# Costava/heightmap-ray-marcher

Measured on AMD Instinct MI355X. Metric: ray-steps/s at 3840x2160, 4096^2 heightmap, higher is better.
Workload: dtype f64; 1 GPU; C3: 4096x4096 heightmap, 3840x2160, spherical hfov 180, step_dist 0.25, grid_width 1; ray_steps_per_frame=1197030646, rays_per_frame=8294400, hits_per_frame=1006074, parallelism=1 GPU, launches back to back on one stream

## Files before the change

### heightmap-ray-marcher_amd/__init__.py

```python
from .lib import (
    Camera, Config, HmrmError, Scene, SceneParams, Stats,
    Ray, RayHit, TraceParams, SegmentParams, Sun, Water, CellMapParams, CellRect, GeometryPlanes, LightPlanes, MAP_TOWARDS_POINT, MAP_WEIGHT, MAP_DIFFUSE, MAP_NO_SHADOWS, RAY_END, TRACE_INTERIOR, SHADE_DIFFUSE, SHADE_NO_SHADOWS, RAY_DTYPE, RAY_HIT_DTYPE, RAY_MISS, RAY_HIT, RAY_CAPPED, MAX_RAYS, as_rays,
    PERSPECTIVE, SPHERICAL, ORTHOGRAPHIC, NEAREST, BILINEAR, NEAREST_F32,
    HMRM_OK, HMRM_E_ARG, HMRM_E_IO, HMRM_E_IMAGE, HMRM_E_CONFIG, HMRM_E_DEVICE, HMRM_E_NOTERM,
    EXPORTED_SYMBOLS, LIB_PATH, NO_PROBE, AA_FACTORS, aa_flags,
    band_local_rows, debug_frame, degrees_to_rads, device_count, image_load, image_load_memory, kernel_src_sha,
    last_error, mip_layout, level_state, calibrate, pick_kernel, plan_order, rcp_error, orbit_camera, orbit_frame_owner, png_encode, record_orbit, record_orbit_multi, record_orbit_shaded, record_orbit_baked, record_orbit_water, LIGHT_U8, LIGHT_U16, WATER_OWN_COLOR, WATER_BAKED, Haze, HAZE_SKY, HAZE_LINEAR, HAZE_EXP, HAZE_EXP2, MAX_HAZE_ENTRIES, haze_table, MAX_VIEWS, camera_array, views_tables, shade_flags, map_flags, sky_directions, render_multi, set_device, write_png, write_ppm, write_pfm,
)
from . import synth
```

### heightmap-ray-marcher_amd/csrc/api_aux.cpp

```cpp
#include <algorithm>
#include <cstdlib>
#include <cstring>
#include <fstream>
#include <new>
#include <sstream>

#include "api_internal.hpp"
#include "config.hpp"
#include "host_pool.hpp"
#include "image_io.hpp"

struct hmrm_config {
	hmrm::Config cfg;
	std::string log_cache, warn_cache;
};

extern "C" {

int hmrm_debug_kernel_choice(const hmrm_scene *s) {
	if (!s) return fail(HMRM_E_ARG, "NULL argument");
	std::lock_guard<std::mutex> lk(const_cast<hmrm_scene *>(s)->mu);
	if (s->knobs.kernel != 0) return s->knobs.kernel;
	return s->choice.use_group ? (s->choice.with_records ? 3 : 1) : 0;
}
// ... 335 lines not shown
	if (cam->projection == HMRM_SPHERICAL) {
		double *cc = tables, *cs = tables + W, *rs = tables + 2 * W, *rc2 = tables + 2 * W + H;
		const int nc = cam->width, nr = cam->height;
		hmrm::parallel_ranges(nc + nr, 1024, [&](int b, int e) {
			if (b < nc) hmrm::fill_col_tables(hc, b, std::min(e, nc), cc, cs);
			if (e > nc) hmrm::fill_row_tables(hc, std::max(b, nc) - nc, e - nc, rs, rc2);
		});
	}
	double *o = out25;
	for (int i = 0; i < 3; ++i) *o++ = f.cam[i];
	for (int i = 0; i < 3; ++i) *o++ = f.upper_left[i];
	for (int i = 0; i < 3; ++i) *o++ = f.plane_right[i];
	for (int i = 0; i < 3; ++i) *o++ = f.plane_down[i];
	for (int i = 0; i < 3; ++i) *o++ = f.look[i];
	for (int i = 0; i < 3; ++i) *o++ = f.c0[i];
	for (int i = 0; i < 3; ++i) *o++ = f.c1[i];
	*o++ = f.nudge;
	*o++ = f.step_dist;
	*o++ = (double)f.grid_pow2;
	*o++ = f.inv_grid_width;
	return HMRM_OK;
}

int hmrm_debug_pick_kernel(int32_t forced, int32_t use_other, int32_t records_ok, int32_t scene_verdict, int32_t scene_with_records,
                           int32_t *with_records_after) {
	hmrm::KernelChoice choice;
	choice.use_group = scene_verdict != 0;
	choice.probed = choice.use_group;
	choice.with_records = scene_with_records != 0;
	const int k = hmrm::pick_fast_kernel(forced, use_other != 0, records_ok != 0, choice);
	if (with_records_after) *with_records_after = choice.with_records ? 1 : 0;
	return k;
}

int hmrm_debug_level_state(int32_t level, int32_t young, int32_t min_level, int32_t out[8]) {
	if (!out || level < 0 || level > hmrm::kMipLevels || min_level < 0 || min_level >= hmrm::kMipLevels)
		return fail(HMRM_E_ARG, "hmrm_debug_level_state: bad argument");
	const uint32_t b = (uint32_t)(hmrm::level_state_table() >> (8 * level)) & 0xffu;
	const int hs = (int)(b & 31u), back = (int)(b >> 5);
	const int lstep = hmrm::level_step(young ? 0 : -1);
	out[0] = hs;
	out[1] = back;
	out[2] = (back + 1) << hs;
	out[3] = lstep;
	out[4] = hmrm::level_coarser(level, lstep);
	out[5] = hmrm::level_finer(level, lstep, min_level);
// ... 31 lines not shown
```

### heightmap-ray-marcher_amd/csrc/api_internal.hpp

```cpp
#pragma once
#include <hip/hip_runtime_api.h>

#include <cstddef>
#include <cstdint>
#include <mutex>
#include <string>
#include <vector>

#include "../../include/hmrm.h"
#include "frame.hpp"
#include "launch_order.hpp"
#include "render.hpp"

#pragma GCC visibility push(hidden)
namespace hmrm {
extern thread_local std::string g_error;
int fail(int code, const std::string &msg);
}
using namespace hmrm;

#define HIP_TRY(expr)                                                                         \
	do {                                                                                      \
		hipError_t e_ = (expr);                                                               \
		if (e_ != hipSuccess)                                                                 \
			return fail(HMRM_E_DEVICE, std::string(#expr) + ": " + hipGetErrorString(e_));    \
	} while (0)

struct Knobs {
	int64_t step_cap = (int64_t)1 << 26;
	int kernel = 0;
	bool tile_order = true;
	int order_mode = 2;
	int diag_mode = 0;
	int min_level = -1;
	int finest_pause = -1;
	bool order_verbose = false;
	bool try_group = true;
	int min_plane_shift = 0;
	int seg_n = 0;
	int seg_b[3] = {0, 0, 0}, seg_c[3] = {0, 0, 0};
};

template <bool kPinned> struct Scratch {
	void *ptr = nullptr;
	size_t cap = 0;
	int reserve(size_t bytes) {
		if (bytes <= cap) return HMRM_OK;
		release();
		if (kPinned) HIP_TRY(hipHostMalloc(&ptr, bytes, hipHostMallocDefault));
		else HIP_TRY(hipMalloc(&ptr, bytes));
		cap = bytes;
		return HMRM_OK;
	}
	template <class T> T *as() const { return static_cast<T *>(ptr); }
	void release() {
		if (ptr) (void)(kPinned ? hipHostFree(ptr) : hipFree(ptr));
		ptr = nullptr;
		cap = 0;
	}
};
using DeviceScratch = Scratch<false>;
using PinnedScratch = Scratch<true>;

constexpr int kFrameSlots = 64;
constexpr int kMaxMeasRows = 512;
constexpr int kProbeAfterFrames = 6;
constexpr int kMaxStreamCtx = 32;

struct FrameSlot {
	bool valid = false;
	uint64_t stamp = 0;
	hmrm_camera cam{};
	hmrm_scene_params params{};
	uint64_t thr_max_bits = 0;
	hmrm::DevFrame frame{};
	std::vector<float> row_cost;
	double *d_tables = nullptr;
	double *h_tables = nullptr;
	hipEvent_t uploaded = nullptr;
	hmrm::OrderCalibration cal;
	int meas_rows = 0;
	hipEvent_t measured = nullptr;
};

struct ViewStage {
	double *h = nullptr, *h_dev = nullptr;
	size_t cap = 0;
	hipEvent_t uploaded = nullptr;
	bool used = false;
	uint64_t stamp = 0;
};
constexpr int kViewStages = 4;
constexpr size_t kMaxViewStagingBytes = (size_t)256 << 20;
struct RetiredArena {
	void *ptr;
	hipEvent_t after;
};

struct StreamCtx {
// ... 177 lines not shown
```

### heightmap-ray-marcher_amd/csrc/api_launch.cpp

```cpp
#include <algorithm>
#include <cstdio>
#include <cstring>

#include "api_internal.hpp"
#include "host_pool.hpp"

static_assert(sizeof(hmrm_sun) == 48, "hmrm_sun has padding");
static_assert(sizeof(hmrm_camera) == 3 * sizeof(int32_t) + 4 + 8 * sizeof(double), "hmrm_camera has padding");
static_assert(sizeof(hmrm_scene_params) == 6 * sizeof(double), "hmrm_scene_params has padding");
static_assert(HMRM_SHADE_DIFFUSE == hmrm::kShadeDiffuse && HMRM_SHADE_NO_SHADOWS == hmrm::kShadeNoShadows, "route_frame's flag bits");

namespace {

int ensure_meas(StreamCtx *c) {
	if (!c->d_meas) HIP_TRY(hipMalloc((void **)&c->d_meas, (size_t)kMaxMeasRows * hmrm::kMeasureStride * sizeof(unsigned long long)));
	if (!c->h_meas) {
		const size_t n = (size_t)kFrameSlots * 2 * kMaxMeasRows * sizeof(unsigned long long);
		HIP_TRY(hipHostMalloc((void **)&c->h_meas, n, hipHostMallocMapped));
		HIP_TRY(hipHostGetDevicePointer((void **)&c->h_meas_dev, c->h_meas, 0));
	}
	return HMRM_OK;
}

bool others_idle(hmrm_scene *s, StreamCtx *c) {
// ... 65 lines not shown
	s->choice.with_records = records_ok;
	if (records_ok) {
		const int rc_r = ensure_records(s);
		if (rc_r) return rc_r;
	}
	hmrm::FrameLaunch l = frame_launch(s, c, f, measured, req);
	for (int pass = 0; pass < 2; ++pass) {
		HIP_TRY(hmrm::launch_measure_init(measured.measure, tiles_y, c->stream));
		l.d_counters = c->d_counters + (pass ? 8 : 0);
		HIP_TRY(hmrm::launch_frame_march(l, pass == 0 ? hmrm::kLeaps : (records_ok ? hmrm::kRecords : hmrm::kPlainGroups)));
		HIP_TRY(hmrm::launch_measure_readback(measured.measure, s->h_probe_dev + (size_t)pass * 2 * kMaxMeasRows, tiles_y, c->stream));
	}
	HIP_TRY(hipEventRecord(s->probe_done, c->stream));
	s->probe_pending = true;
	s->choice.probed = true;
	s->probe_rows = tiles_y;
	s->probe_epoch_launched = s->probe_epoch;
	s->probe_ctx = c;
	c->probe_in_flight = true;
	return raise_measure_fence(s, c);
}

int launch_kernel(hmrm_scene *s, StreamCtx *c, const hmrm::DevFrame &f, const hmrm::RowMap &rows_in_order, const FrameRequest &req,
                  bool use_group) {
	const bool huge_side = s->map_w >= (1 << 24) || s->map_h >= (1 << 24);
	const LitFrame *lit = req.lit;
	const hmrm::FrameRoute route = hmrm::route_frame(s->knobs.kernel, huge_side, f.sampling, f.aa_shift != 0, req.interior == Interior::kByKernels,
	                                                 lit != nullptr, lit ? lit->shade_flags : 0u, lit && lit->sum);
	if (route.refused) return fail(HMRM_E_ARG, "maps with a side of 2^24 cells or more support nearest sampling only");
	hmrm::FrameLaunch l = frame_launch(s, c, f, rows_in_order, req);
	l.family = route.family;
	if (lit) {
		l.sun = lit->sun;
		if (route.ambient_sun) l.sun.ambient = 255u;
		l.primary_interior = lit->primary_interior;
		if (lit->sum) l.lsum = *lit->sum;
	}
	if (req.geom) {
		l.family = hmrm::kFrameGeometry;
		l.geo = *req.geom;
		l.primary_interior = req.interior != Interior::kNot;
	}
	if (req.baked) {
		l.family = hmrm::kFrameBaked;
		l.baked = *req.baked;
		l.primary_interior = req.interior != Interior::kNot;
	}
	if (req.water) {
		const bool aa = f.aa_shift != 0;
		if (req.baked) l.family = aa ? hmrm::kFrameWaterBakedAA : hmrm::kFrameWaterBaked;
		else l.family = aa ? hmrm::kFrameWaterAA : hmrm::kFrameWater;
		l.water = *req.water;
		l.primary_interior = req.interior != Interior::kNot;
		if (req.water_sun) {
// ... 8 lines not shown
	}
	if (route.literal) {
		HIP_TRY(hmrm::launch_frame_literal(l));
		return HMRM_OK;
	}
	const hmrm::FastKernel k = (hmrm::FastKernel)hmrm::pick_fast_kernel(s->knobs.kernel, use_group, f.sampling == 0 && s->d_records, s->choice);
	if (k == hmrm::kRecords) {
		const int rc_r = ensure_records(s);
		if (rc_r) return rc_r;
	}
	HIP_TRY(hmrm::launch_frame_march(l, k));
	return HMRM_OK;
}

int launch_maybe_measured(hmrm_scene *s, StreamCtx *c, const hmrm::DevFrame &f, FrameSlot *slot, hmrm::RowMap &rows_in_order, int tiles_y,
                          bool measure_now, const FrameRequest &req, bool use_group) {
	if (measure_now) {
		const int rc_m = ensure_meas(c);
		if (rc_m) return rc_m;
		if (!slot->measured) HIP_TRY(hipEventCreateWithFlags(&slot->measured, hipEventDisableTiming));
		rows_in_order.measure = c->d_meas;
		HIP_TRY(hmrm::launch_measure_init(rows_in_order.measure, tiles_y, c->stream));
	}
	const int rc_k = launch_kernel(s, c, f, rows_in_order, req, use_group);
	if (rc_k || !measure_now) return rc_k;
	const size_t idx = (size_t)(slot - c->slots);
	HIP_TRY(hmrm::launch_measure_readback(rows_in_order.measure, c->h_meas_dev + idx * 2 * kMaxMeasRows, tiles_y, c->stream));
	HIP_TRY(hipEventRecord(slot->measured, c->stream));
	slot->meas_rows = tiles_y;
	c->meas_owner = slot;
	return raise_measure_fence(s, c);
}

}

namespace hmrm {

int check_camera(const hmrm_camera *cam) {
	if (!cam) return fail(HMRM_E_ARG, "camera is NULL");
	if (cam->width <= 0 || cam->height <= 0) return fail(HMRM_E_ARG, "resolution must be positive");
	if ((int64_t)cam->width * cam->height > ((int64_t)1 << 31) / 4)
		return fail(HMRM_E_ARG, "resolution too large (the reference indexes the framebuffer with int)");
	if (cam->projection < 1 || cam->projection > 3) return fail(HMRM_E_ARG, "projection must be 1, 2 or 3");
	if (cam->sampling > HMRM_NEAREST_F32) return fail(HMRM_E_ARG, "sampling must be 0 (nearest), 1 (bilinear) or 2 (nearest, float heights)");
	return HMRM_OK;
}

// ... 67 lines not shown
		}
		hmrm::DevFrame &fr = slot->frame;
		hmrm::build_frame(hc, s->map_w, s->map_h, s->params.min_height, s->params.max_height, s->params.grid_width,
		                  &fr, nullptr, nullptr, nullptr, nullptr);
		if (cam->projection == HMRM_SPHERICAL) {
			const FrameSlot *row_donor = nullptr, *col_donor = nullptr;
			for (const FrameSlot &o : c->slots) {
				if (!o.valid || &o == slot || o.cam.projection != HMRM_SPHERICAL || !o.h_tables) continue;
				if (o.cam.width != cam->width || o.cam.hfov != cam->hfov) continue;
				if (!col_donor && o.cam.hang == cam->hang) col_donor = &o;
				if (!row_donor && o.cam.height == cam->height && o.cam.vang == cam->vang) row_donor = &o;
			}
			if (col_donor) memcpy(cc, col_donor->h_tables, 2 * W * sizeof(double));
			if (row_donor) memcpy(rs, row_donor->h_tables + 2 * (size_t)row_donor->cam.width, 2 * H * sizeof(double));
			const int nc = col_donor ? 0 : cam->width, nr = row_donor ? 0 : cam->height;
			if (nc + nr > 0)
				hmrm::parallel_ranges(nc + nr, 1024, [&](int b, int e) {
					if (b < nc) hmrm::fill_col_tables(hc, b, std::min(e, nc), cc, cs);
					if (e > nc) hmrm::fill_row_tables(hc, std::max(b, nc) - nc, e - nc, rs, rc);
				});
		}
		slot->row_cost.assign(((size_t)cam->height + kCostRows - 1) / kCostRows, 0.0f);
		hmrm::estimate_row_costs(fr, cc, cs, rs, rc, kCostRows, slot->row_cost.data());
		if (cam->projection == HMRM_SPHERICAL) {
			HIP_TRY(hmrm::launch_upload_tables(c->h_arena_dev + (slot->h_tables - c->h_arena), slot->d_tables, 2 * W + 2 * H, c->stream));
			HIP_TRY(hipEventRecord(slot->uploaded, c->stream));
			fr.col_cos_ha = slot->d_tables;
			fr.col_sin_ha = slot->d_tables + W;
			fr.row_sin_va = slot->d_tables + 2 * W;
			fr.row_cos_va = slot->d_tables + 2 * W + H;
		}
		if (cam->sampling == HMRM_BILINEAR) {
			const int rc2 = ensure_bilinear_pyramid(s);
			if (rc2 != HMRM_OK) return rc2;
		}
		finish_frame_record(s, cam->sampling, &fr);
		slot->cam = *cam;
		slot->params = s->params;
		slot->thr_max_bits = thr_bits;
		slot->valid = true;
		for (size_t k = s->settled.size(); k-- > 0;) {
			const hmrm_scene::SettledOrder &so = s->settled[k];
			if (memcmp(&so.cam, cam, sizeof *cam) != 0 || memcmp(&so.params, &s->params, sizeof s->params) != 0 || so.thr_max_bits != thr_bits) continue;
			slot->cal.adopt(so.order);
			break;
		}
	}
// ... 167 lines not shown
```

### heightmap-ray-marcher_amd/csrc/api_scene.cpp

```cpp
#include <cstdio>
#include <cstdlib>
#include <cstring>
#include <new>
#include <vector>

#include "api_internal.hpp"

namespace hmrm {

thread_local std::string g_error;

int fail(int code, const std::string &msg) {
	g_error = msg;
	return code;
}

int set_error(int code, const char *msg) { return fail(code, msg ? msg : ""); }

}

namespace {

Knobs read_knobs() {
	Knobs k;
	if (const char *s = getenv("HMRM_STEP_CAP")) {
		const long long v = atoll(s);
		if (v > 0) k.step_cap = v > 0x7fffffffLL ? 0x7fffffffLL : (int64_t)v;
	}
	if (const char *s = getenv("HMRM_KERNEL")) k.kernel = strcmp(s, "simple") == 0 ? 2 : (strcmp(s, "group") == 0 ? 1 : (strcmp(s, "rec") == 0 ? 3 : 0));
	if (const char *s = getenv("HMRM_TILE_ORDER")) {
		k.tile_order = s[0] != '0';
		if (s[0] == '1' || s[0] == '2') k.order_mode = s[0] - '0';
	}
	if (const char *s = getenv("HMRM_DIAG_ITERS")) k.diag_mode = atoi(s);
	if (const char *s = getenv("HMRM_ORDER_VERBOSE")) k.order_verbose = s[0] == '1';
	if (const char *s = getenv("HMRM_TRY_GROUP")) k.try_group = s[0] != '0';
	if (const char *s = getenv("HMRM_TILE_SEGMENTS")) {
		int b = 0, c = 0, used = 0;
		while (k.seg_n < 3 && sscanf(s, "%d:%d%n", &b, &c, &used) == 2 && b >= 0 && c > 0) {
			k.seg_b[k.seg_n] = b;
			k.seg_c[k.seg_n] = c;
			++k.seg_n;
			s += used;
			if (*s != ',') break;
			++s;
		}
	}
	if (const char *s = getenv("HMRM_DEBUG_PLANE_SHIFT")) {
		const int v = atoi(s);
		if (v > 0 && v <= 28) k.min_plane_shift = v;
	}
	if (const char *s = getenv("HMRM_MIN_LEVEL"))
		if (s[0] >= '0' && s[0] < '0' + hmrm::kMipLevels) k.min_level = s[0] - '0';
	if (const char *s = getenv("HMRM_FINEST_PAUSE"))
		if (s[0] >= '0' && s[0] <= '9') k.finest_pause = s[0] - '0';
	return k;
}

void destroy_ctx(StreamCtx *c) {
// ... 424 lines not shown
```

### heightmap-ray-marcher_amd/csrc/camera.cpp

```cpp
#include "frame.hpp"

#include <cmath>
#include <cstring>

namespace hmrm {
namespace {

struct Vec3 {
	double x, y, z;
};
inline Vec3 operator+(Vec3 a, Vec3 b) { return Vec3{a.x + b.x, a.y + b.y, a.z + b.z}; }
inline Vec3 operator-(Vec3 a, Vec3 b) { return Vec3{a.x - b.x, a.y - b.y, a.z - b.z}; }
inline Vec3 operator-(Vec3 a) { return Vec3{-a.x, -a.y, -a.z}; }
inline Vec3 operator*(double s, Vec3 v) { return Vec3{s * v.x, s * v.y, s * v.z}; }
inline Vec3 cross(Vec3 a, Vec3 b) {
	return Vec3{a.y * b.z - b.y * a.z, a.z * b.x - b.z * a.x, a.x * b.y - b.x * a.y};
}
inline double dot(Vec3 a, Vec3 b) {
	const double px = a.x * b.x, py = a.y * b.y, pz = a.z * b.z;
	return px + py + pz;
}
inline Vec3 normalize(Vec3 v) {
	const double inv = 1.0 / std::sqrt(dot(v, v));
	return Vec3{v.x * inv, v.y * inv, v.z * inv};
// ... 105 lines not shown
		store(f->plane_down, (cam.height * ow) * (-u));
	}

	fill_scene_fields(map_w, map_h, min_height, max_height, grid_width, cam.step_dist, f);

	for (int i = 0; i < 3; ++i) {
		auto high = [](double v) {
			uint64_t b;
			memcpy(&b, &v, sizeof b);
			return (uint32_t)(b >> 32);
		};
		const uint32_t h0 = high(f->c0[i] - cam.pos[i]), h1 = high(f->c1[i] - cam.pos[i]);
		const bool moderate = (((h0 >> 20) & 0x7ffu) - 523u) < 1000u && (((h1 >> 20) & 0x7ffu) - 523u) < 1000u;
		f->box_side_known[i] = (moderate && ((h0 ^ h1) >> 31) == 0u) ? 1 : 0;
		f->box_side[i] = f->box_side_known[i] ? h0 : 0u;
	}

	const double cells_per_step = std::fabs(cam.step_dist / grid_width);
	f->min_window = cells_per_step > 0.35 ? 16 : 4;
	f->finest_pause = cells_per_step > 0.35 ? 6 : 0;
	f->min_level = 0;
}

}
```

### heightmap-ray-marcher_amd/csrc/frame.hpp

```cpp
#pragma once
#include <stdint.h>

namespace hmrm {

struct DevFrame {
	int32_t screen_w, screen_h;
	int32_t projection;
	int32_t map_w, map_h;
	uint8_t bg[4];
	double cam[3];
	double upper_left[3], plane_right[3], plane_down[3];
	double look[3];
	const double *col_cos_ha, *col_sin_ha;
	const double *row_sin_va, *row_cos_va;
	double c0[3], c1[3];
	double grid_width;
	double nudge;
	double step_dist;
	double inv_grid_width;
	int32_t grid_pow2;
	int32_t grid_mode;
	double thr_max;
	int64_t step_cap;
	const float *mipbuf;
// ... 203 lines not shown
constexpr int kMaxHazeEntries = 4096;

struct HostCamera {
	int32_t width, height, projection;
	uint8_t bg_r, bg_g, bg_b, sampling;
	double hfov, hang, vang, pos[3], ortho_width, step_dist;
};

void build_frame(const HostCamera &cam, int32_t map_w, int32_t map_h,
                 double min_height, double max_height, double grid_width,
                 DevFrame *out,
                 double *col_cos_ha, double *col_sin_ha,
                 double *row_sin_va, double *row_cos_va);

void fill_scene_fields(int32_t map_w, int32_t map_h, double min_height, double max_height, double grid_width,
                       double step_dist, DevFrame *out);

void fill_col_tables(const HostCamera &cam, int32_t begin, int32_t end, double *col_cos_ha, double *col_sin_ha);
void fill_row_tables(const HostCamera &cam, int32_t begin, int32_t end, double *row_sin_va, double *row_cos_va);

void estimate_row_costs(const DevFrame &f, const double *col_cos_ha, const double *col_sin_ha,
                        const double *row_sin_va, const double *row_cos_va, int rows_per_sample, float *out);

}
```

### heightmap-ray-marcher_amd/csrc/render.hpp

```cpp
#pragma once
#include <hip/hip_runtime_api.h>
#include <stdint.h>

#include "frame.hpp"
#include "march_dispatch.hpp"

namespace hmrm {

hipError_t launch_prepare_heights(const uint8_t *d_rgb, double *d_out, int64_t n, double lum_r,
                                  double lum_g, double lum_b, double min_h, double max_h, bool plain,
                                  unsigned long long *d_max_key, hipStream_t stream);
double max_key_to_double(unsigned long long key);

struct FrameLaunch {
	const double *d_thr;
	const float *d_thr32;
	const uint32_t *d_cmap;
	const WindowRecord *d_records;
	uint32_t *d_out;
	int64_t out_stride_px;
	unsigned long long *d_counters;
	uint32_t *d_steps;
	double *d_entry;
	bool stats;
	const DevFrame &f;
	const RowMap &rows;
	FrameFamily family;
	SunRules sun;
	bool primary_interior;
	GeomPlanes geo;
	hipStream_t stream;
	LightSum lsum = LightSum{nullptr, nullptr, 0, 0, 0u};
	BakedLight baked = BakedLight{nullptr, 0u};
	WaterRules water = WaterRules{0.0, 0.0, 0u, 0u, 0u, 0u};
	HazeRules haze = HazeRules{nullptr, 0.0, 0.0, 0u, 0u, 0u};
	const DevFrame *d_frames = nullptr;
	int32_t n_views = 0;
	int64_t view_stride_px = 0;
};
hipError_t launch_frame_march(const FrameLaunch &l, FastKernel kernel);
hipError_t launch_frame_literal(const FrameLaunch &l);
hipError_t launch_trace_rays(const DevFrame &f, const double *d_thr, const float *d_thr32, const uint32_t *d_cmap,
                             const RayBatch &batch, unsigned long long *d_counters, FastKernel kernel,
                             const WindowRecord *d_records, hipStream_t stream);
hipError_t launch_trace_rays_literal(const DevFrame &f, const double *d_thr, const uint32_t *d_cmap, const RayBatch &batch,
                                     unsigned long long *d_counters, hipStream_t stream);
hipError_t launch_trace_segments(const DevFrame &f, const double *d_thr, const float *d_thr32, const uint32_t *d_cmap,
                                 const RayBatch &batch, const SegRules &seg, unsigned long long *d_counters, FastKernel kernel,
                                 const WindowRecord *d_records, hipStream_t stream);
hipError_t launch_trace_segments_literal(const DevFrame &f, const double *d_thr, const uint32_t *d_cmap, const RayBatch &batch,
                                         const SegRules &seg, unsigned long long *d_counters, hipStream_t stream);
hipError_t launch_cell_map(const DevFrame &f, const double *d_thr, const float *d_thr32, uint8_t *d_out, int64_t stride_bytes,
                           const CellRules &cells, unsigned long long *d_counters, FastKernel kernel, const WindowRecord *d_records,
                           hipStream_t stream);
hipError_t launch_cell_map_literal(const DevFrame &f, const double *d_thr, uint8_t *d_out, int64_t stride_bytes, const CellRules &cells,
                                   unsigned long long *d_counters, hipStream_t stream);
hipError_t launch_cell_map_sum(const DevFrame &f, const double *d_thr, const float *d_thr32, uint16_t *d_out, int64_t stride_bytes,
                               const CellRules &cells, const CellSums &sums, unsigned long long *d_counters, FastKernel kernel,
                               const WindowRecord *d_records, hipStream_t stream);
hipError_t launch_cell_map_sum_literal(const DevFrame &f, const double *d_thr, uint16_t *d_out, int64_t stride_bytes,
                                       const CellRules &cells, const CellSums &sums, unsigned long long *d_counters, hipStream_t stream);
// ... 24 lines not shown
```

### heightmap-ray-marcher_amd/csrc/render_fast.hip

```cpp
#ifdef HMRM_TIMELINE
#include <cstdio>
#include <cstdlib>
#endif
#include "march_frame.hpp"

namespace hmrm {

#ifdef HMRM_TIMELINE
struct TimelineRec { unsigned long long t0, t1; unsigned int xcc, pad; };
__device__ TimelineRec *g_timeline = nullptr;
__device__ __forceinline__ void timeline_wave_done(unsigned long long t0) {
	if (!g_timeline || (threadIdx.x & 63) != 0) return;
	unsigned xcc;
	asm volatile("s_getreg_b32 %0, hwreg(HW_REG_XCC_ID)" : "=s"(xcc));
	const size_t wave = ((size_t)(blockIdx.z * gridDim.y + blockIdx.y) * gridDim.x + blockIdx.x) * (kBlockThreads / 64) + (threadIdx.x >> 6);
	g_timeline[wave] = TimelineRec{t0, (unsigned long long)__builtin_amdgcn_s_memrealtime(), xcc, 0u};
}
static void timeline_before_launch(dim3 grid, int tiles_y, const RowMap &rows) {
	static TimelineRec *host = nullptr, *devbuf = nullptr;
	static size_t cap = 0, used = 0;
	static int gx = 0, gy = 0, ty = 0, segs[7] = {0, 0, 0, 0, 0, 0, 0};
	const size_t waves = (size_t)grid.x * grid.y * grid.z * (kBlockThreads / 64);
	if (waves > cap) {
		(void)hipDeviceSynchronize();
// ... 199 lines not shown
}
hipError_t launch_measure_init(unsigned long long *d_rec, int tile_rows, hipStream_t stream) {
	const int n = tile_rows * kMeasureStride;
	hipLaunchKernelGGL(k_measure_init, dim3((unsigned)((n + 255) / 256)), dim3(256), 0, stream, d_rec, n);
	return hipGetLastError();
}
hipError_t launch_measure_readback(const unsigned long long *d_rec, unsigned long long *h_pinned_dev, int tile_rows, hipStream_t stream) {
	hipLaunchKernelGGL(k_measure_readback, dim3((unsigned)((tile_rows + 255) / 256)), dim3(256), 0, stream, d_rec, h_pinned_dev, tile_rows);
	return hipGetLastError();
}

__global__ __launch_bounds__(256) void k_thr_to_float(const double *__restrict__ thr, float *__restrict__ dst, int64_t n) {
	const int64_t stride = (int64_t)gridDim.x * blockDim.x;
	for (int64_t i = (int64_t)blockIdx.x * blockDim.x + threadIdx.x; i < n; i += stride) dst[i] = (float)thr[i];
}

hipError_t launch_thr_to_float(const double *d_thr, float *d_thr32, int64_t n, hipStream_t stream) {
	int64_t blocks = (n + 255) / 256;
	if (blocks > 256 * 16) blocks = 256 * 16;
	hipLaunchKernelGGL(k_thr_to_float, dim3((unsigned)(blocks < 1 ? 1 : blocks)), dim3(256), 0, stream, d_thr, d_thr32, n);
	return hipGetLastError();
}

hipError_t launch_render_fast(const FrameLaunch &l, FastKernel kernel) {
	return launch_fast<false>(l.f, l.rows, l.d_thr, l.d_thr32, l.d_cmap, l.d_out, l.out_stride_px, l.d_counters, l.d_steps, l.d_entry,
	                          l.stats, kernel, l.d_records, l.stream);
}

hipError_t launch_frame_march(const FrameLaunch &l, FastKernel kernel) {
	const bool aa = l.f.aa_shift != 0;
	switch (l.family) {
	case kFrameInterior: return launch_render_interior(l, kernel);
	case kFrameLit: return aa ? launch_render_lit_aa(l, kernel) : launch_render_lit(l, kernel);
	case kFrameShaded: return aa ? launch_render_shaded_aa(l, kernel) : launch_render_shaded(l, kernel);
	case kFrameLitShaded: return aa ? launch_render_lit_shaded_aa(l, kernel) : launch_render_lit_shaded(l, kernel);
	case kFrameGeometry: return launch_render_geometry(l, kernel);
	case kFrameLitSum: return launch_render_lit_sum(l, kernel);
	case kFrameBaked: return aa ? launch_render_baked_aa(l, kernel) : launch_render_baked(l, kernel);
	case kFrameWater: return launch_render_water(l, kernel);
	case kFrameWaterAA: return launch_render_water_aa(l, kernel);
	case kFrameWaterBaked: return launch_render_water_baked(l, kernel);
	case kFrameWaterBakedAA: return launch_render_water_baked_aa(l, kernel);
	case kFrameWaterLit: return launch_render_water_lit(l, kernel);
	case kFrameHaze: return aa ? launch_render_haze_aa(l, kernel) : launch_render_haze(l, kernel);
	case kFrameViews: return launch_render_views(l, kernel);
	default: return aa ? launch_render_fast_aa(l, kernel) : launch_render_fast(l, kernel);
	}
// ... 9 lines not shown
```

### heightmap-ray-marcher_amd/lib.py

```python
from __future__ import annotations

import ctypes as C
import os

import numpy as np

_HERE = os.path.dirname(os.path.abspath(__file__))
LIB_PATH = os.path.join(_HERE, "libhmrm.so")

HMRM_OK = 0
HMRM_E_ARG, HMRM_E_IO, HMRM_E_IMAGE, HMRM_E_CONFIG, HMRM_E_DEVICE, HMRM_E_NOTERM = -1, -2, -3, -4, -5, -6
PERSPECTIVE, SPHERICAL, ORTHOGRAPHIC = 1, 2, 3
NEAREST, BILINEAR, NEAREST_F32 = 0, 1, 2
_PROJ_NAMES = {"perspective": 1, "spherical": 2, "orthographic": 3}


NO_PROBE = 1
AA_FACTORS = (1, 2, 4, 8)


def aa_flags(n: int) -> int:
    return (int(n) & 15) << 8


# ... 230 lines not shown
    u8p, dp, u32p = C.POINTER(C.c_uint8), C.POINTER(C.c_double), C.POINTER(C.c_uint32)
    vp, i32 = C.c_void_p, C.c_int32
    sig = {
        "hmrm_abi_version": (C.c_int, []),
        "hmrm_last_error": (C.c_char_p, []),
        "hmrm_device_count": (C.c_int, []),
        "hmrm_set_device": (C.c_int, [C.c_int]),
        "hmrm_scene_create": (C.c_int, [vp, vp, i32, i32, C.POINTER(SceneParams), C.POINTER(vp)]),
        "hmrm_scene_update": (C.c_int, [vp, C.POINTER(SceneParams)]),
        "hmrm_scene_destroy": (None, [vp]),
        "hmrm_scene_read_heights": (C.c_int, [vp, vp]),
        "hmrm_render": (C.c_int, [vp, C.POINTER(Camera), vp, C.c_size_t]),
        "hmrm_render_cycle": (C.c_int, [vp, C.POINTER(Camera), vp, C.c_size_t, i32, i32]),
        "hmrm_render_multi": (C.c_int, [C.POINTER(vp), i32, C.POINTER(Camera), vp, C.c_size_t]),
        "hmrm_render_rows_device": (C.c_int, [vp, C.POINTER(Camera), vp, C.c_size_t, i32, i32, i32, i32, i32, vp]),
        "hmrm_scene_take_capped": (C.c_int, [vp, vp, C.POINTER(C.c_uint64)]),
        "hmrm_debug_reload_env": (C.c_int, [vp]),
        "hmrm_debug_kernel_choice": (C.c_int, [vp]),
        "hmrm_debug_read_records": (C.c_int, [vp, vp, vp]),
        "hmrm_debug_pick_kernel": (C.c_int, [i32, i32, i32, i32, i32, C.POINTER(i32)]),
        "hmrm_debug_calibrate": (C.c_int, [vp, i32, i32, i32, i32, i32, vp, vp, vp, vp, C.POINTER(i32), C.POINTER(i32), C.POINTER(i32), C.POINTER(i32)]),
        "hmrm_debug_mip_layout": (C.c_int, [i32, i32, C.POINTER(i32), C.POINTER(i32), C.POINTER(i32)]),
        "hmrm_debug_level_state": (C.c_int, [i32, i32, i32, C.POINTER(i32)]),
        "hmrm_band_local_rows": (i32, [i32, i32, i32, i32]),
        "hmrm_render_stats": (C.c_int, [vp, C.POINTER(Camera), vp, C.c_size_t, C.POINTER(Stats), vp, vp]),
        "hmrm_render_aa": (C.c_int, [vp, C.POINTER(Camera), i32, vp, C.c_size_t, C.POINTER(Stats)]),
        "hmrm_trace_rays": (C.c_int, [vp, C.POINTER(TraceParams), vp, C.c_int64, vp, C.POINTER(Stats)]),
        "hmrm_trace_rays_device": (C.c_int, [vp, C.POINTER(TraceParams), vp, C.c_int64, vp, vp]),
        "hmrm_trace_segments": (C.c_int, [vp, C.POINTER(SegmentParams), vp, vp, C.c_int64, vp, C.POINTER(Stats)]),
        "hmrm_trace_segments_device": (C.c_int, [vp, C.POINTER(SegmentParams), vp, vp, C.c_int64, vp, vp]),
        "hmrm_cell_map": (C.c_int, [vp, C.POINTER(CellMapParams), C.POINTER(CellRect), vp, C.c_size_t]),
        "hmrm_cell_map_device": (C.c_int, [vp, C.POINTER(CellMapParams), C.POINTER(CellRect), vp, C.c_size_t, vp]),
        "hmrm_cell_map_sum": (C.c_int, [vp, C.POINTER(CellMapParams), dp, i32, C.POINTER(CellRect), vp, C.c_size_t]),
        "hmrm_cell_map_sum_device": (C.c_int, [vp, C.POINTER(CellMapParams), vp, i32, C.POINTER(CellRect), vp, C.c_size_t, vp]),
        "hmrm_sky_directions": (C.c_int, [i32, i32, dp]),
        "hmrm_render_geometry": (C.c_int, [vp, C.POINTER(Camera), C.POINTER(GeometryPlanes)]),
        "hmrm_render_geometry_device": (C.c_int, [vp, C.POINTER(Camera), C.POINTER(GeometryPlanes), vp]),
        "hmrm_render_lit_sum": (C.c_int, [vp, C.POINTER(Camera), C.POINTER(Sun), dp, i32, C.c_uint32, C.POINTER(LightPlanes)]),
        "hmrm_render_lit_sum_device": (C.c_int, [vp, C.POINTER(Camera), C.POINTER(Sun), vp, i32, C.c_uint32, C.POINTER(LightPlanes), vp]),
        "hmrm_render_interior": (C.c_int, [vp, C.POINTER(Camera), vp, C.c_size_t]),
        "hmrm_render_lit": (C.c_int, [vp, C.POINTER(Camera), C.POINTER(Sun), vp, C.c_size_t]),
        "hmrm_render_water": (C.c_int, [vp, C.POINTER(Camera), C.POINTER(Water), vp, C.c_size_t]),
        "hmrm_render_water_device": (C.c_int, [vp, C.POINTER(Camera), C.POINTER(Water), vp, C.c_size_t, vp]),
        "hmrm_render_water_lit": (C.c_int, [vp, C.POINTER(Camera), C.POINTER(Water), C.POINTER(Sun), C.c_uint32, vp, C.c_size_t]),
        "hmrm_render_water_lit_device": (C.c_int, [vp, C.POINTER(Camera), C.POINTER(Water), C.POINTER(Sun), C.c_uint32, vp, C.c_size_t, vp]),
        "hmrm_render_water_aa": (C.c_int, [vp, C.POINTER(Camera), C.POINTER(Water), C.c_uint32, i32, vp, C.c_size_t]),
# ... 152 lines not shown


def _check(rc: int, allow=()):
    if rc != HMRM_OK and rc not in allow:
        raise HmrmError(rc, last_error())
    return rc


def _ptr(a: np.ndarray):
    return a.ctypes.data_as(C.c_void_p)


def device_count() -> int:
    n = lib.hmrm_device_count()
    if n < 0:
        raise HmrmError(n, last_error())
    return n


def set_device(i: int):
    _check(lib.hmrm_set_device(int(i)))


_ENV_KNOBS = ("HMRM_KERNEL", "HMRM_STEP_CAP", "HMRM_TILE_ORDER", "HMRM_DIAG_ITERS", "HMRM_MIN_LEVEL", "HMRM_FINEST_PAUSE", "HMRM_TILE_SEGMENTS", "HMRM_ORDER_VERBOSE", "HMRM_TRY_GROUP")


def shade_flags(diffuse=True, shadows=True) -> int:
    return (SHADE_DIFFUSE if diffuse else 0) | (0 if shadows else SHADE_NO_SHADOWS)


def map_flags(point=False, weight=False, diffuse=False, shadows=True) -> int:
    return ((MAP_TOWARDS_POINT if point else 0) | (MAP_WEIGHT if weight else 0) | (MAP_DIFFUSE if diffuse else 0)
            | (0 if shadows else MAP_NO_SHADOWS))


def sky_directions(rings: int, per_ring: int) -> np.ndarray:
    n = int(rings) * int(per_ring)
    out = np.zeros((max(min(n, 256), 1), 3), dtype=np.float64)
    rc = lib.hmrm_sky_directions(int(rings), int(per_ring), out.ctypes.data_as(C.POINTER(C.c_double)))
    if rc < 0:
        raise HmrmError(rc, last_error())
    return out[:rc]


def _as_rect(rect):
    if rect is None or isinstance(rect, CellRect):
        return rect
# ... 457 lines not shown

    def bench_kernel_ms(self, cam: Camera, iters: int) -> float:
        self._sync_env()
        ms = lib.hmrm_bench_kernel_ms(self._h, C.byref(cam), int(iters))
        if ms < 0:
            raise HmrmError(HMRM_E_DEVICE, last_error())
        return ms


def debug_frame(cam: Camera, params: SceneParams, map_w: int, map_h: int):
    out = np.empty(25, dtype=np.float64)
    tables = np.empty(2 * cam.width + 2 * cam.height, dtype=np.float64)
    _check(lib.hmrm_debug_frame(C.byref(cam), C.byref(params), map_w, map_h, _ptr(out), _ptr(tables)))
    W, H = cam.width, cam.height
    rec = {"cam": out[0:3], "upper_left": out[3:6], "plane_right": out[6:9], "plane_down": out[9:12],
           "look": out[12:15], "c0": out[15:18], "c1": out[18:21], "nudge": out[21], "step_dist": out[22],
           "grid_pow2": int(out[23]), "inv_grid_width": out[24]}
    if cam.projection == SPHERICAL:
        rec.update(col_cos_ha=tables[0:W], col_sin_ha=tables[W:2 * W],
                   row_sin_va=tables[2 * W:2 * W + H], row_cos_va=tables[2 * W + H:])
    return rec


def mip_layout(map_w: int, map_h: int):
    row, shift, levels = C.c_int32(), C.c_int32(), C.c_int32()
    rc = lib.hmrm_debug_mip_layout(int(map_w), int(map_h), C.byref(row), C.byref(shift), C.byref(levels))
    if rc < 0:
        raise HmrmError(rc, last_error())
    return row.value, shift.value, levels.value, bool(rc)


def level_state(level: int, young: bool, min_level: int):
    out = (C.c_int32 * 8)()
    rc = lib.hmrm_debug_level_state(int(level), int(bool(young)), int(min_level), out)
    if rc < 0:
        raise HmrmError(rc, last_error())
    keys = ("stride_shift", "back", "cells", "lstep", "coarser", "finer", "at_finest", "byte")
    return dict(zip(keys, (int(v) for v in out))), int(rc)


def pick_kernel(forced=0, use_other=False, records_ok=True, verdict=False, verdict_with_records=False):
    after = C.c_int32()
    k = lib.hmrm_debug_pick_kernel(int(forced), int(use_other), int(records_ok), int(verdict), int(verdict_with_records), C.byref(after))
    return int(k), bool(after.value)


# ... 340 lines not shown
```

### include/hmrm.h

```cpp
#ifndef HMRM_H
#define HMRM_H

#include <stddef.h>
#include <stdint.h>

#ifdef __cplusplus
extern "C" {
#endif

#define HMRM_ABI_VERSION 1

enum {
	HMRM_OK          =  0,
	HMRM_E_ARG       = -1,
	HMRM_E_IO        = -2,
	HMRM_E_IMAGE     = -3,
	HMRM_E_CONFIG    = -4,
	HMRM_E_DEVICE    = -5,
	HMRM_E_NOTERM    = -6
};

enum {
	HMRM_PERSPECTIVE  = 1,
	HMRM_SPHERICAL    = 2,
// ... 279 lines not shown
int hmrm_render_views(const hmrm_scene *scene, const hmrm_camera *cams, int32_t n, uint32_t flags,
                      uint8_t *rgba, size_t stride_bytes, size_t view_stride_bytes);
int hmrm_render_views_device(const hmrm_scene *scene, const hmrm_camera *cams, int32_t n, uint32_t flags,
                             void *d_rgba, size_t stride_bytes, size_t view_stride_bytes, void *hip_stream);
int hmrm_debug_views_tables(const hmrm_camera *cams, int32_t n, int32_t *out_col_index, int32_t *out_row_index);

int hmrm_pick(const hmrm_scene *scene, const hmrm_camera *cam, int32_t px, int32_t py, hmrm_ray_hit *hit);

int hmrm_debug_ray(const hmrm_scene *scene, const hmrm_camera *cam,
                   int32_t px, int32_t py, double pos[3], double dir[3], double *entry_d);

int hmrm_debug_frame(const hmrm_camera *cam, const hmrm_scene_params *params,
                     int32_t map_w, int32_t map_h, double *out25, double *tables);

int hmrm_debug_plan_order(const uint64_t *records, int32_t tile_rows, int32_t rot, int32_t pieces_begin[3],
                          int32_t pieces_count[3], int32_t *tile_row_of_grid_row);

int hmrm_debug_calibrate(const uint64_t *records, int32_t launches, int32_t tile_rows, int32_t rot, int32_t may_probe,
                         int32_t scene_already_probed, const uint8_t *can_measure, int32_t *trial_used, int32_t *measured,
                         int32_t *group_kernel, int32_t *n_trials, int32_t *best, int32_t *scene_use_group,
                         int32_t *settled_at_launch);

int hmrm_debug_level_state(int32_t level, int32_t young, int32_t min_level, int32_t out[8]);

int hmrm_debug_rcp_error(int32_t mode, uint64_t count, uint64_t seed, int32_t exp_lo, int32_t exp_hi,
                         double *max_rel_err, uint64_t *hist64);

int hmrm_debug_mip_layout(int32_t map_w, int32_t map_h, int32_t *mip_row, int32_t *plane_shift, int32_t *levels);

int hmrm_debug_kernel_choice(const hmrm_scene *scene);

int hmrm_debug_read_records(const hmrm_scene *scene, void *records_out, double *thr_out);

int hmrm_debug_pick_kernel(int32_t forced, int32_t use_other, int32_t records_ok, int32_t scene_verdict, int32_t scene_with_records,
                           int32_t *with_records_after);

int hmrm_debug_reload_env(hmrm_scene *scene);

double hmrm_last_kernel_ms(void);

double hmrm_bench_kernel_ms(const hmrm_scene *scene, const hmrm_camera *cam, int32_t iters);

void hmrm_orbit_camera(const hmrm_camera *base, double centre_x, double centre_y, double radius,
                       double hang0, int32_t frame, int32_t frames, hmrm_camera *out);
int hmrm_record_orbit(const hmrm_scene *scene, const hmrm_camera *base, double centre_x, double centre_y,
                      double radius, double hang0, int32_t frames, const char *dir, long long id,
// ... 81 lines not shown
```

Baseline: 12550 billion ray-steps/s.

## Skip marching for spherical columns whose rays point away from the heightmap box

```diff
diff --git a/heightmap-ray-marcher_amd/__init__.py b/heightmap-ray-marcher_amd/__init__.py
--- a/heightmap-ray-marcher_amd/__init__.py
+++ b/heightmap-ray-marcher_amd/__init__.py
@@ -4,7 +4,7 @@
     PERSPECTIVE, SPHERICAL, ORTHOGRAPHIC, NEAREST, BILINEAR, NEAREST_F32,
     HMRM_OK, HMRM_E_ARG, HMRM_E_IO, HMRM_E_IMAGE, HMRM_E_CONFIG, HMRM_E_DEVICE, HMRM_E_NOTERM,
     EXPORTED_SYMBOLS, LIB_PATH, NO_PROBE, AA_FACTORS, aa_flags,
-    band_local_rows, debug_frame, degrees_to_rads, device_count, image_load, image_load_memory, kernel_src_sha,
+    band_local_rows, debug_frame, debug_away, degrees_to_rads, device_count, image_load, image_load_memory, kernel_src_sha,
     last_error, mip_layout, level_state, calibrate, pick_kernel, plan_order, rcp_error, orbit_camera, orbit_frame_owner, png_encode, record_orbit, record_orbit_multi, record_orbit_shaded, record_orbit_baked, record_orbit_water, LIGHT_U8, LIGHT_U16, WATER_OWN_COLOR, WATER_BAKED, Haze, HAZE_SKY, HAZE_LINEAR, HAZE_EXP, HAZE_EXP2, MAX_HAZE_ENTRIES, haze_table, MAX_VIEWS, camera_array, views_tables, shade_flags, map_flags, sky_directions, render_multi, set_device, write_png, write_ppm, write_pfm,
 )
 from . import synth
diff --git a/heightmap-ray-marcher_amd/csrc/api_aux.cpp b/heightmap-ray-marcher_amd/csrc/api_aux.cpp
--- a/heightmap-ray-marcher_amd/csrc/api_aux.cpp
+++ b/heightmap-ray-marcher_amd/csrc/api_aux.cpp
@@ -381,6 +381,34 @@
 	return HMRM_OK;
 }
 
+int hmrm_debug_away(const hmrm_camera *cam, const hmrm_scene_params *params, int32_t map_w, int32_t map_h, double *tables,
+                    uint8_t *col_away, uint8_t *row_away, int32_t out10[10]) {
+	int rc = check_camera(cam);
+	if (rc) return rc;
+	if (!params || !tables || !col_away || !row_away || !out10) return fail(HMRM_E_ARG, "NULL argument");
+	if (cam->projection != HMRM_SPHERICAL) return fail(HMRM_E_ARG, "hmrm_debug_away: spherical cameras only");
+	double rec[25];
+	if ((rc = hmrm_debug_frame(cam, params, map_w, map_h, rec, tables))) return rc;
+	hmrm::HostCamera hc;
+	to_host_camera(cam, &hc);
+	hmrm::DevFrame f;
+	hmrm::build_frame(hc, map_w, map_h, params->min_height, params->max_height, params->grid_width, &f, nullptr, nullptr, nullptr, nullptr);
+	const size_t W = (size_t)cam->width, H = (size_t)cam->height;
+	int tile_w = 1, tile_h = 1;
+	hmrm::render_tile_shape(&tile_w, &tile_h);
+	hmrm::AwaySplit aw;
+	hmrm::classify_away(f, tile_w, tables, tables + W, tables + 2 * W, tables + 2 * W + H, col_away, row_away, &aw);
+	out10[0] = aw.on;
+	out10[1] = aw.tx0;
+	out10[2] = aw.tx1;
+	out10[3] = aw.tiles_x;
+	for (int i = 0; i < 3; ++i) {
+		out10[4 + i] = (int32_t)f.box_side[i];
+		out10[7 + i] = f.box_side_known[i];
+	}
+	return tile_w;
+}
+
 int hmrm_debug_pick_kernel(int32_t forced, int32_t use_other, int32_t records_ok, int32_t scene_verdict, int32_t scene_with_records,
                            int32_t *with_records_after) {
 	hmrm::KernelChoice choice;
diff --git a/heightmap-ray-marcher_amd/csrc/api_internal.hpp b/heightmap-ray-marcher_amd/csrc/api_internal.hpp
--- a/heightmap-ray-marcher_amd/csrc/api_internal.hpp
+++ b/heightmap-ray-marcher_amd/csrc/api_internal.hpp
@@ -39,6 +39,7 @@
 	int min_plane_shift = 0;
 	int seg_n = 0;
 	int seg_b[3] = {0, 0, 0}, seg_c[3] = {0, 0, 0};
+	bool miss_fill = true;
 };
 
 template <bool kPinned> struct Scratch {
@@ -75,6 +76,7 @@
 	uint64_t thr_max_bits = 0;
 	hmrm::DevFrame frame{};
 	std::vector<float> row_cost;
+	hmrm::AwaySplit away{};
 	double *d_tables = nullptr;
 	double *h_tables = nullptr;
 	hipEvent_t uploaded = nullptr;
diff --git a/heightmap-ray-marcher_amd/csrc/api_launch.cpp b/heightmap-ray-marcher_amd/csrc/api_launch.cpp
--- a/heightmap-ray-marcher_amd/csrc/api_launch.cpp
+++ b/heightmap-ray-marcher_amd/csrc/api_launch.cpp
@@ -111,7 +111,7 @@
 }
 
 int launch_kernel(hmrm_scene *s, StreamCtx *c, const hmrm::DevFrame &f, const hmrm::RowMap &rows_in_order, const FrameRequest &req,
-                  bool use_group) {
+                  bool use_group, const hmrm::AwaySplit &away) {
 	const bool huge_side = s->map_w >= (1 << 24) || s->map_h >= (1 << 24);
 	const LitFrame *lit = req.lit;
 	const hmrm::FrameRoute route = hmrm::route_frame(s->knobs.kernel, huge_side, f.sampling, f.aa_shift != 0, req.interior == Interior::kByKernels,
@@ -119,6 +119,7 @@
 	if (route.refused) return fail(HMRM_E_ARG, "maps with a side of 2^24 cells or more support nearest sampling only");
 	hmrm::FrameLaunch l = frame_launch(s, c, f, rows_in_order, req);
 	l.family = route.family;
+	if (s->knobs.miss_fill) l.away = away;
 	if (lit) {
 		l.sun = lit->sun;
 		if (route.ambient_sun) l.sun.ambient = 255u;
@@ -173,7 +174,7 @@
 		rows_in_order.measure = c->d_meas;
 		HIP_TRY(hmrm::launch_measure_init(rows_in_order.measure, tiles_y, c->stream));
 	}
-	const int rc_k = launch_kernel(s, c, f, rows_in_order, req, use_group);
+	const int rc_k = launch_kernel(s, c, f, rows_in_order, req, use_group, slot->away);
 	if (rc_k || !measure_now) return rc_k;
 	const size_t idx = (size_t)(slot - c->slots);
 	HIP_TRY(hmrm::launch_measure_readback(rows_in_order.measure, c->h_meas_dev + idx * 2 * kMaxMeasRows, tiles_y, c->stream));
@@ -287,7 +288,11 @@
 		}
 		slot->row_cost.assign(((size_t)cam->height + kCostRows - 1) / kCostRows, 0.0f);
 		hmrm::estimate_row_costs(fr, cc, cs, rs, rc, kCostRows, slot->row_cost.data());
+		slot->away = hmrm::AwaySplit{0, 0, 0, 0};
 		if (cam->projection == HMRM_SPHERICAL) {
+			int tile_w = 1, tile_h = 1;
+			hmrm::render_tile_shape(&tile_w, &tile_h);
+			hmrm::classify_away(fr, tile_w, cc, cs, rs, rc, nullptr, nullptr, &slot->away);
 			HIP_TRY(hmrm::launch_upload_tables(c->h_arena_dev + (slot->h_tables - c->h_arena), slot->d_tables, 2 * W + 2 * H, c->stream));
 			HIP_TRY(hipEventRecord(slot->uploaded, c->stream));
 			fr.col_cos_ha = slot->d_tables;
diff --git a/heightmap-ray-marcher_amd/csrc/api_scene.cpp b/heightmap-ray-marcher_amd/csrc/api_scene.cpp
--- a/heightmap-ray-marcher_amd/csrc/api_scene.cpp
+++ b/heightmap-ray-marcher_amd/csrc/api_scene.cpp
@@ -35,6 +35,7 @@
 	if (const char *s = getenv("HMRM_DIAG_ITERS")) k.diag_mode = atoi(s);
 	if (const char *s = getenv("HMRM_ORDER_VERBOSE")) k.order_verbose = s[0] == '1';
 	if (const char *s = getenv("HMRM_TRY_GROUP")) k.try_group = s[0] != '0';
+	if (const char *s = getenv("HMRM_MISS_FILL")) k.miss_fill = s[0] != '0';
 	if (const char *s = getenv("HMRM_TILE_SEGMENTS")) {
 		int b = 0, c = 0, used = 0;
 		while (k.seg_n < 3 && sscanf(s, "%d:%d%n", &b, &c, &used) == 2 && b >= 0 && c > 0) {
diff --git a/heightmap-ray-marcher_amd/csrc/camera.cpp b/heightmap-ray-marcher_amd/csrc/camera.cpp
--- a/heightmap-ray-marcher_amd/csrc/camera.cpp
+++ b/heightmap-ray-marcher_amd/csrc/camera.cpp
@@ -151,4 +151,58 @@
 	f->min_level = 0;
 }
 
-}
+void classify_away(const DevFrame &f, int tile_w, const double *col_cos_ha, const double *col_sin_ha, const double *row_sin_va,
+                   const double *row_cos_va, uint8_t *col_away, uint8_t *row_away, AwaySplit *out) {
+	auto high = [](double v) {
+		uint64_t b;
+		memcpy(&b, &v, sizeof b);
+		return (uint32_t)(b >> 32);
+	};
+	const int W = f.screen_w, H = f.screen_h;
+	const int tiles_x = (W + tile_w - 1) / tile_w;
+	*out = AwaySplit{0, 0, tiles_x, tiles_x};
+	if (col_away) memset(col_away, 0, (size_t)W);
+	if (row_away) memset(row_away, 0, (size_t)H);
+	if (f.projection != 2 || W <= 0 || H <= 0) return;
+
+	if (row_away && f.box_side_known[2])
+		for (int py = 0; py < H; ++py) {
+			const uint32_t hd = high(row_cos_va[py]);
+			row_away[py] = ((((hd >> 20) & 0x7ffu) - 523u) < 1000u && ((f.box_side[2] ^ hd) >> 31) != 0u) ? 1 : 0;
+		}
+
+	uint32_t e_lo = 0x7ffu, e_hi = 0u, sign_or = 0u, sign_and = 1u;
+	for (int py = 0; py < H; ++py) {
+		const uint32_t hs = high(row_sin_va[py]), e = (hs >> 20) & 0x7ffu;
+		e_lo = e < e_lo ? e : e_lo;
+		e_hi = e > e_hi ? e : e_hi;
+		sign_or |= hs >> 31;
+		sign_and &= hs >> 31;
+	}
+	if (e_lo == 0u || e_hi == 0x7ffu || sign_or != sign_and) return;
+	const uint32_t sva_sign = sign_or;
+	auto product_away = [&](double v, int axis) {
+		if (!f.box_side_known[axis]) return false;
+		const uint32_t hv = high(v), e = (hv >> 20) & 0x7ffu;
+		if (e == 0u || e == 0x7ffu) return false;
+		const int lo = (int)e_lo + (int)e - 1023, hi = (int)e_hi + (int)e - 1022;
+		if (lo < 523 || hi > 1522) return false;
+		return (((f.box_side[axis] >> 31) ^ (hv >> 31) ^ sva_sign) & 1u) != 0u;
+	};
+	int hot0 = tiles_x, hot1 = 0;
+	for (int px = 0; px < W; ++px) {
+		const bool away = product_away(col_cos_ha[px], 0) || product_away(col_sin_ha[px], 1);
+		if (col_away) col_away[px] = away ? 1 : 0;
+		if (!away) {
+			const int t = px / tile_w;
+			hot0 = t < hot0 ? t : hot0;
+			hot1 = t + 1 > hot1 ? t + 1 : hot1;
+		}
+	}
+	if (hot1 <= hot0) hot0 = hot1 = 0;
+	out->tx0 = hot0;
+	out->tx1 = hot1;
+	out->on = (hot0 > 0 || hot1 < tiles_x) ? 1 : 0;
+}
+
+}
diff --git a/heightmap-ray-marcher_amd/csrc/frame.hpp b/heightmap-ray-marcher_amd/csrc/frame.hpp
--- a/heightmap-ray-marcher_amd/csrc/frame.hpp
+++ b/heightmap-ray-marcher_amd/csrc/frame.hpp
@@ -249,4 +249,21 @@
 void estimate_row_costs(const DevFrame &f, const double *col_cos_ha, const double *col_sin_ha,
                         const double *row_sin_va, const double *row_cos_va, int rows_per_sample, float *out);
 
-}
+struct AwaySplit {
+	int32_t on;
+	int32_t tx0, tx1;
+	int32_t tiles_x;
+};
+void classify_away(const DevFrame &f, int tile_w, const double *col_cos_ha, const double *col_sin_ha, const double *row_sin_va,
+                   const double *row_cos_va, uint8_t *col_away, uint8_t *row_away, AwaySplit *out);
+struct MissFill {
+	int32_t tx0;
+	int32_t march_rows;
+	int32_t left_px, right_begin, n_away;
+	int32_t spans;
+	int32_t n_blocks;
+	int32_t wide;
+};
+constexpr int kFillRows = 8, kFillLanePx = 4;
+
+}
diff --git a/heightmap-ray-marcher_amd/csrc/render.hpp b/heightmap-ray-marcher_amd/csrc/render.hpp
--- a/heightmap-ray-marcher_amd/csrc/render.hpp
+++ b/heightmap-ray-marcher_amd/csrc/render.hpp
@@ -37,6 +37,7 @@
 	const DevFrame *d_frames = nullptr;
 	int32_t n_views = 0;
 	int64_t view_stride_px = 0;
+	AwaySplit away = AwaySplit{0, 0, 0, 0};
 };
 hipError_t launch_frame_march(const FrameLaunch &l, FastKernel kernel);
 hipError_t launch_frame_literal(const FrameLaunch &l);
diff --git a/heightmap-ray-marcher_amd/csrc/render_fast.hip b/heightmap-ray-marcher_amd/csrc/render_fast.hip
--- a/heightmap-ray-marcher_amd/csrc/render_fast.hip
+++ b/heightmap-ray-marcher_amd/csrc/render_fast.hip
@@ -245,7 +245,89 @@
 	return hipGetLastError();
 }
 
+__device__ __forceinline__ void fill_away_block(const DevFrame &f, const RowMap &rows, uint32_t *__restrict__ out, int64_t out_stride_px,
+                                                const MissFill &fill, unsigned block) {
+	if (block >= (unsigned)fill.n_blocks) return;
+	const unsigned group = block / (unsigned)fill.spans, span = block - group * (unsigned)fill.spans;
+	const int a = (int)(span * (unsigned)(kBlockThreads * kFillLanePx) + threadIdx.x * (unsigned)kFillLanePx);
+	if (a >= fill.n_away) return;
+	const int px = a < fill.left_px ? a : a - fill.left_px + fill.right_begin;
+	const bool whole = fill.wide != 0 && px + kFillLanePx <= f.screen_w;
+#pragma unroll
+	for (int r = 0; r < kFillRows; ++r) {
+		const int lrow = (int)group * kFillRows + r;
+		if (lrow >= rows.local_rows) break;
+		const int py = frame_row_of(rows, lrow);
+		if (py >= f.screen_h) continue;
+		const uint32_t rgba = shade_miss(f, f.row_cos_va[py]);
+		uint32_t *dst = out + ((uint64_t)(uint32_t)lrow * (uint64_t)out_stride_px + (uint32_t)px);
+		static_assert(kFillLanePx == 4, "one 16-byte store per lane and row");
+		if (whole) *reinterpret_cast<uint4 *>(dst) = make_uint4(rgba, rgba, rgba, rgba);
+		else {
+#pragma unroll
+			for (int k = 0; k < kFillLanePx; ++k)
+				if (px + k < f.screen_w) dst[k] = rgba;
+		}
+	}
+}
+
+template <int GWM, int LEAP, int SAMP>
+__global__ __launch_bounds__(kBlockThreads, HMRM_MIN_WAVES) HMRM_OCCUPANCY_ATTR void k_render_fast_split(
+    const DevFrame f, const RowMap rows, const double *__restrict__ thr, const uint32_t *__restrict__ cmap, uint32_t *__restrict__ out,
+    int64_t out_stride_px, int tiles_y, StatsOut st, const MissFill fill) {
+	if (blockIdx.y >= (unsigned)fill.march_rows) {
+		fill_away_block(f, rows, out, out_stride_px, fill, (blockIdx.y - (unsigned)fill.march_rows) * gridDim.x + blockIdx.x);
+		return;
+	}
+	unsigned long long wave_t0 = 0;
+	if (rows.measure) wave_t0 = __builtin_amdgcn_s_memrealtime();
+	const int tile_y = render_wave_tile<Family<FramesOf<false, false>, 2, GWM, LEAP, SAMP>>(
+	    f, rows, thr, cmap, out, out_stride_px, tiles_y, st, (int)blockIdx.x + fill.tx0, blockIdx.y, (int)(threadIdx.x >> 6),
+	    (int)(threadIdx.x & 63));
+	if (rows.measure && tile_y >= 0 && (threadIdx.x & 63) == 0) {
+		const unsigned long long took = __builtin_amdgcn_s_memrealtime() - wave_t0;
+		unsigned long long *rec = rows.measure + (size_t)tile_y * kMeasureStride;
+		if (blockIdx.x == 0 && threadIdx.x == 0) rec[0] = wave_t0;
+		atomicMax(&rec[1 + (blockIdx.x & 31u)], took);
+	}
+}
+
+static hipError_t launch_fast_split(const FrameLaunch &l, FastKernel kernel) {
+	const LaunchGrid g = tile_grid(l.f, l.rows);
+	if (g.tiles_y == 0) return g.err;
+	const AwaySplit &aw = l.away;
+	MissFill fill;
+	fill.tx0 = aw.tx0;
+	fill.march_rows = aw.tx1 > aw.tx0 ? g.tiles_y : 0;
+	fill.left_px = aw.tx0 * kTileW;
+	fill.right_begin = aw.tx1 * kTileW < l.f.screen_w ? aw.tx1 * kTileW : l.f.screen_w;
+	fill.n_away = fill.left_px + (l.f.screen_w - fill.right_begin);
+	constexpr int span_px = kBlockThreads * kFillLanePx;
+	fill.spans = (fill.n_away + span_px - 1) / span_px;
+	const int64_t n_blocks = (int64_t)((l.rows.local_rows + kFillRows - 1) / kFillRows) * fill.spans;
+	const unsigned gx = aw.tx1 > aw.tx0 ? (unsigned)(aw.tx1 - aw.tx0) : 32u;
+	const int64_t fill_rows = (n_blocks + gx - 1) / gx;
+	if (g.grid.z != 1u || fill.n_away <= 0 || n_blocks > 0x7fffffff || fill.march_rows + fill_rows > 65535)
+		return launch_fast<false>(l.f, l.rows, l.d_thr, l.d_thr32, l.d_cmap, l.d_out, l.out_stride_px, l.d_counters, l.d_steps, l.d_entry,
+		                          l.stats, kernel, l.d_records, l.stream);
+	fill.n_blocks = (int32_t)n_blocks;
+	fill.wide = ((uintptr_t)l.d_out % 16u == 0 && l.out_stride_px % 4 == 0) ? 1 : 0;
+	DevFrame fr = l.f;
+	const double *d_thr = nullptr;
+	if (const hipError_t e = select_tables(&fr, kernel, l.d_thr, l.d_thr32, l.d_records, &d_thr); e != hipSuccess) return e;
+	const StatsOut st{l.d_counters, l.d_steps, l.d_entry};
+	const dim3 grid(gx, (unsigned)(fill.march_rows + fill_rows), 1u);
+	dispatch_march(l.f.grid_mode, kernel, l.f.sampling, [&](auto gwm, auto leap, auto samp) {
+		if constexpr (leap() != kPlainGroups)
+			hipLaunchKernelGGL((k_render_fast_split<gwm(), leap(), samp()>), grid, dim3(kBlockThreads), 0, l.stream, fr, l.rows, d_thr, l.d_cmap,
+			                   l.d_out, l.out_stride_px, g.tiles_y, st, fill);
+	});
+	return hipGetLastError();
+}
+
 hipError_t launch_render_fast(const FrameLaunch &l, FastKernel kernel) {
+	if (l.away.on && kernel != kPlainGroups && !l.stats && l.f.projection == 2 && l.f.aa_shift == 0 && l.d_out != nullptr)
+		return launch_fast_split(l, kernel);
 	return launch_fast<false>(l.f, l.rows, l.d_thr, l.d_thr32, l.d_cmap, l.d_out, l.out_stride_px, l.d_counters, l.d_steps, l.d_entry,
 	                          l.stats, kernel, l.d_records, l.stream);
 }
diff --git a/heightmap-ray-marcher_amd/lib.py b/heightmap-ray-marcher_amd/lib.py
--- a/heightmap-ray-marcher_amd/lib.py
+++ b/heightmap-ray-marcher_amd/lib.py
@@ -276,6 +276,7 @@
         "hmrm_debug_calibrate": (C.c_int, [vp, i32, i32, i32, i32, i32, vp, vp, vp, vp, C.POINTER(i32), C.POINTER(i32), C.POINTER(i32), C.POINTER(i32)]),
         "hmrm_debug_mip_layout": (C.c_int, [i32, i32, C.POINTER(i32), C.POINTER(i32), C.POINTER(i32)]),
         "hmrm_debug_level_state": (C.c_int, [i32, i32, i32, C.POINTER(i32)]),
+        "hmrm_debug_away": (C.c_int, [C.POINTER(Camera), C.POINTER(SceneParams), i32, i32, vp, vp, vp, C.POINTER(i32)]),
         "hmrm_band_local_rows": (i32, [i32, i32, i32, i32]),
         "hmrm_render_stats": (C.c_int, [vp, C.POINTER(Camera), vp, C.c_size_t, C.POINTER(Stats), vp, vp]),
         "hmrm_render_aa": (C.c_int, [vp, C.POINTER(Camera), i32, vp, C.c_size_t, C.POINTER(Stats)]),
@@ -474,7 +475,7 @@
     _check(lib.hmrm_set_device(int(i)))
 
 
-_ENV_KNOBS = ("HMRM_KERNEL", "HMRM_STEP_CAP", "HMRM_TILE_ORDER", "HMRM_DIAG_ITERS", "HMRM_MIN_LEVEL", "HMRM_FINEST_PAUSE", "HMRM_TILE_SEGMENTS", "HMRM_ORDER_VERBOSE", "HMRM_TRY_GROUP")
+_ENV_KNOBS = ("HMRM_KERNEL", "HMRM_STEP_CAP", "HMRM_TILE_ORDER", "HMRM_DIAG_ITERS", "HMRM_MIN_LEVEL", "HMRM_FINEST_PAUSE", "HMRM_TILE_SEGMENTS", "HMRM_ORDER_VERBOSE", "HMRM_TRY_GROUP", "HMRM_MISS_FILL")
 
 
 def shade_flags(diffuse=True, shadows=True) -> int:
@@ -978,6 +979,20 @@
     return rec
 
 
+def debug_away(cam: Camera, params: SceneParams, map_w: int, map_h: int):
+    W, H = cam.width, cam.height
+    tables = np.empty(2 * W + 2 * H, dtype=np.float64)
+    col, row = np.zeros(W, dtype=np.uint8), np.zeros(H, dtype=np.uint8)
+    out = (C.c_int32 * 10)()
+    tile_w = lib.hmrm_debug_away(C.byref(cam), C.byref(params), map_w, map_h, _ptr(tables), _ptr(col), _ptr(row), out)
+    if tile_w < 0:
+        raise HmrmError(tile_w, last_error())
+    return {"col_away": col.astype(bool), "row_away": row.astype(bool), "on": bool(out[0]), "tx0": int(out[1]), "tx1": int(out[2]),
+            "tiles_x": int(out[3]), "tile_w": int(tile_w), "box_side": [int(out[4 + i]) & 0xffffffff for i in range(3)],
+            "box_side_known": [bool(out[7 + i]) for i in range(3)],
+            "col_cos_ha": tables[0:W], "col_sin_ha": tables[W:2 * W], "row_sin_va": tables[2 * W:2 * W + H], "row_cos_va": tables[2 * W + H:]}
+
+
 def mip_layout(map_w: int, map_h: int):
     row, shift, levels = C.c_int32(), C.c_int32(), C.c_int32()
     rc = lib.hmrm_debug_mip_layout(int(map_w), int(map_h), C.byref(row), C.byref(shift), C.byref(levels))
diff --git a/include/hmrm.h b/include/hmrm.h
--- a/include/hmrm.h
+++ b/include/hmrm.h
@@ -325,6 +325,9 @@
                          int32_t *settled_at_launch);
 
 int hmrm_debug_level_state(int32_t level, int32_t young, int32_t min_level, int32_t out[8]);
+
+int hmrm_debug_away(const hmrm_camera *cam, const hmrm_scene_params *params, int32_t map_w, int32_t map_h, double *tables,
+                    uint8_t *col_away, uint8_t *row_away, int32_t out10[10]);
 
 int hmrm_debug_rcp_error(int32_t mode, uint64_t count, uint64_t seed, int32_t exp_lo, int32_t exp_hi,
                          double *max_rel_err, uint64_t *hist64);
```

Measured after the change: 13070 billion ray-steps/s, median of 3. 1.04x the previous value.
